# Streampunk/phaneron

Hardware: AMD Instinct MI355X
Metric: frames/sec, 4-layer 2160p50 composite pipeline (v210 unpack->CSC->combine->CSC->v210 pack) (higher is better)
Workload: dtype f32

## Files before the change

phaneron_amd/csrc/ph_kernels_lds.hip:

```cpp
#include "ph_device.h"
#include "ph_kernels.h"
#include "ph_ldslut.h"

#include <cstdlib>

#include <type_traits>

#pragma clang fp contract(off)

#ifndef PH_PROBE
#define PH_PROBE 0
#endif
#if PH_PROBE
__device__ unsigned long long g_fused_probe[2048 * 12];
extern "C" int ph_debug_fused_probe(unsigned long long *out, int n_words) {
  return (int)hipMemcpyFromSymbol(out, HIP_SYMBOL(g_fused_probe), (size_t)n_words * 8);
}
#define PH_STAMP(k)                                                                  \
  do {                                                                               \
    if (threadIdx.x == 0 && tile_begin == wg_begin) {                                \
      g_fused_probe[blockIdx.x * 12 + 2 * (k)] = __builtin_amdgcn_s_memtime();       \
      g_fused_probe[blockIdx.x * 12 + 2 * (k) + 1] = __builtin_amdgcn_s_memrealtime(); \
    }                                                                                \
  } while (0)
#else
#define PH_STAMP(k) do { } while (0)
#endif

#ifndef PH_BALANCE_WAVES
#define PH_BALANCE_WAVES 1
#endif
#if PH_BALANCE_WAVES
__device__ __forceinline__ void ph_set_wave_priority(int level) {
  switch (level) {
    case 3: __builtin_amdgcn_s_setprio(3); break;
    case 2: __builtin_amdgcn_s_setprio(2); break;
    case 1: __builtin_amdgcn_s_setprio(1); break;
    default: __builtin_amdgcn_s_setprio(0); break;
  }
}
#define PH_BALANCE(p) ph_set_wave_priority(3 - ((p) * 4) / P)
#else
#define PH_BALANCE(p) do { } while (0)
#endif

namespace ph {


__device__ __forceinline__ uint4 write_quad_lds(const float (&rgb)[18], const WriteK &wk, const LutK &lut) {
  uint32_t y[6], u[3], v[3];
#pragma unroll
  for (int j = 0; j < 6; ++j) {
    if ((j & 1) == 0) {
      const Yuv1 c = write_px_lds(rgb[3 * j], rgb[3 * j + 1], rgb[3 * j + 2], wk, lut);
      y[j] = c.y, u[j >> 1] = c.u, v[j >> 1] = c.v;
    } else {
      y[j] = write_px_luma_lds(rgb[3 * j], rgb[3 * j + 1], rgb[3 * j + 2], wk, lut);
    }
  }
  return pack_quad(y, u, v);
}

#ifndef PH_FUSED_SPLIT
#define PH_FUSED_SPLIT 0
#endif
template <int N, int P, int BS, bool PIPE = false, int MODE = 0, bool TAIL = false>
__global__ __launch_bounds__(BS) void fused_v210_combine_lds_kernel(FusedLdsArgs a, uint32_t *handoff = nullptr) {
  static_assert(!TAIL || (!PIPE && MODE == 0), "the tail instantiation exists for the shipped form only");
  const ReadK rk = load_read_k(a.f.rd_cm, a.f.rd_gm);
  const WriteK wk = load_write_k(a.f.wr_cm);
  const LutK rlut = make_lut_k(a.rd), wlut = make_lut_k(a.wr);
  const bool std_matrix = ycbcr_matrix_is_standard(rk);
  const uint32_t job = blockIdx.x / a.wg_per_job, wg_in_job = blockIdx.x - job * a.wg_per_job;
  auto layer_ptr = [&](int l) { return reinterpret_cast<const uint4 *>(job ? a.more_layers[job - 1][l] : a.f.layers[l]); };
  uint4 *const out_ptr = reinterpret_cast<uint4 *>(job ? a.more_out[job - 1] : a.f.out);
  const uint32_t per_wg = (a.f.total_quads + a.wg_per_job - 1) / a.wg_per_job;
  const uint32_t wg_begin = wg_in_job * per_wg;
  const uint32_t wg_end = wg_begin + per_wg < a.f.total_quads ? wg_begin + per_wg : a.f.total_quads;
  const uint32_t tile_quads = BS * P;
  for (uint32_t tile_begin = wg_begin; tile_begin < wg_end; tile_begin += tile_quads) {
    uint32_t st[P][9];
    auto quad_of = [&](int p) {
      const uint32_t f = tile_begin + p * BS + threadIdx.x;
      return f < wg_end ? f : wg_end - 1;
    };
    uint4 w = load_stream(layer_ptr(0) + quad_of(0));
    auto slot_kind = [&](uint32_t f) -> uint32_t {
      const uint32_t g = f - __umulhi(f, a.f.magic_qpp) * a.f.quads_per_line_pitch;
      return g < a.f.quads_per_line_used ? 0u : (g == a.f.quads_per_line_used && a.f.tail_px) ? 1u : 2u;
    };
    auto phase1_slice = [&](auto tag, uint4 w, uint32_t f, uint32_t f_next, bool more, uint32_t(&st)[9]) -> uint4 {
      const bool in_tail = TAIL && slot_kind(f) == 1u;
      const float last = TAIL ? (in_tail ? 0.0f : 1.0f) : 1.0f;
      float acc[18];
#pragma unroll
      for (int i = 0; i < 18; ++i) acc[i] = 0.0f;
#pragma unroll 1
      for (int l = 0; l < N; ++l) {
        uint4 nxt = w;
        if (l + 1 < N) nxt = load_stream(layer_ptr(l + 1) + f);
        else if (more) nxt = load_stream(layer_ptr(0) + f_next);
        const Yuv6 q = unpack_quad(w);
#pragma unroll
        for (int j = 0; j < 6; ++j) {
          const float4 t = read_px_lds<decltype(tag)::value>(q.y[j], q.cb[j >> 1], q.cr[j >> 1], rk, rlut, last);
          const float kk = 1.0f - t.w;
          asm volatile("v_fma_f32 %0, %0, %3, %4\n\tv_fma_f32 %1, %1, %3, %5\n\tv_fma_f32 %2, %2, %3, %6"
                       : "+v"(acc[3 * j]), "+v"(acc[3 * j + 1]), "+v"(acc[3 * j + 2])
                       : "v"(kk), "v"(t.x), "v"(t.y), "v"(t.z));
        }
        w = nxt;
      }
#pragma unroll
      for (int i = 0; i < 9; ++i) {
        const uint32_t lo = __float_as_uint(TAIL ? lds_lut_index_unit_tail(acc[2 * i], in_tail) : lds_lut_index_unit(acc[2 * i]));
        const uint32_t hi = __float_as_uint(TAIL ? lds_lut_index_unit_tail(acc[2 * i + 1], in_tail) : lds_lut_index_unit(acc[2 * i + 1]));
        st[i] = __builtin_amdgcn_perm(hi, lo, 0x05040100u);
        asm volatile("" : "+v"(st[i]));
      }
      return w;
    };
    PH_STAMP(0);
    if (MODE == 0 || (MODE == 1 && tile_begin == wg_begin)) {
      lds_lut_load<BS>(a.rd);
      __syncthreads();
    }
    PH_STAMP(1);
    const uint32_t tile_left = wg_end - tile_begin;
    if constexpr (PIPE) {
      auto phase1_all = [&](auto tag) {
        constexpr bool STD = decltype(tag)::value;
        auto issue_first = [&](const uint4 &word) {
          return read_px_issue<STD>((float)((word.x >> 10) & 0x3ff), (float)(word.x & 0x3ff), (float)((word.x >> 20) & 0x3ff), rk, rlut);
        };
        auto issue_px = [&](const uint4 &word, int j) {
          const uint32_t wy = j == 0 ? word.x : j < 3 ? word.y : j == 3 ? word.z : word.w;
          const uint32_t sy = (j == 0 || j == 3) ? 10u : (j == 1 || j == 4) ? 0u : 20u;
          const int pr = j >> 1;
          const uint32_t wcb = pr == 0 ? word.x : pr == 1 ? word.y : word.z, scb = 10u * pr;
          const uint32_t wcr = pr == 0 ? word.x : pr == 1 ? word.z : word.w, scr = pr == 0 ? 20u : pr == 1 ? 0u : 10u;
          return read_px_issue<STD>((float)((wy >> sy) & 0x3ff), (float)((wcb >> scb) & 0x3ff), (float)((wcr >> scr) & 0x3ff), rk, rlut);
        };
        PxPending pend = issue_first(w);
#pragma unroll
        for (int p = 0; p < P; ++p) {
          if (p * BS < tile_left) {
            PH_BALANCE(p);
            const uint32_t f = quad_of(p);
            const bool more = (p + 1 < P) && ((p + 1) * BS < tile_left);
            const uint32_t f_next = more ? quad_of(p + 1) : f;
            float acc[18];
#pragma unroll
            for (int i = 0; i < 18; ++i) acc[i] = 0.0f;
#pragma unroll 1
            for (int l = 0; l < N; ++l) {
              uint4 nxt = w;
              if (l + 1 < N) nxt = load_stream(layer_ptr(l + 1) + f);
              else if (more) nxt = load_stream(layer_ptr(0) + f_next);
#pragma unroll
              for (int j = 0; j < 6; ++j) {
                PxPending nx;
                if (j < 5) nx = issue_px(w, j + 1);
                else {
                  uint4 first = nxt;
                  asm volatile("" : "+v"(first.x));
                  nx = issue_first(first);
                }
                __builtin_amdgcn_sched_barrier(0);
                const float4 t = read_px_finish(pend, rk);
                const float kk = 1.0f - t.w;
                asm volatile("v_fma_f32 %0, %0, %3, %4\n\tv_fma_f32 %1, %1, %3, %5\n\tv_fma_f32 %2, %2, %3, %6"
                             : "+v"(acc[3 * j]), "+v"(acc[3 * j + 1]), "+v"(acc[3 * j + 2])
                             : "v"(kk), "v"(t.x), "v"(t.y), "v"(t.z));
                __builtin_amdgcn_sched_barrier(0);
                pend = nx;
              }
              w = nxt;
            }
#pragma unroll
            for (int i = 0; i < 9; ++i) {
              const uint32_t lo = __float_as_uint(lds_lut_index_unit(acc[2 * i]));
              const uint32_t hi = __float_as_uint(lds_lut_index_unit(acc[2 * i + 1]));
              st[p][i] = __builtin_amdgcn_perm(hi, lo, 0x05040100u);
              asm volatile("" : "+v"(st[p][i]));
            }
          }
        }
      };
      if (std_matrix) phase1_all(std::true_type{});
      else phase1_all(std::false_type{});
      PH_STAMP(2);
      __syncthreads();
      lds_lut_load<BS>(a.wr);
      __syncthreads();
      PH_STAMP(3);
      auto idx_at = [&](int p, int i) {
        const uint32_t v = st[p][i >> 1];
        return __uint_as_float(((i & 1) ? (v >> 16) : (v & 0xFFFFu)) | 0x4B400000u);
      };
      PxPending wp = write_px_issue(idx_at(0, 0), idx_at(0, 1), idx_at(0, 2), wlut);
#pragma unroll
      for (int p = 0; p < P; ++p) {
        if (p * BS < tile_left) {
          PH_BALANCE(p);
          const uint32_t f = tile_begin + p * BS + threadIdx.x;
          uint32_t y[6], u[3], v[3];
#pragma unroll
          for (int j = 0; j < 6; ++j) {
            PxPending nx = wp;
            if (j < 5) nx = write_px_issue(idx_at(p, 3 * j + 3), idx_at(p, 3 * j + 4), idx_at(p, 3 * j + 5), wlut);
            else if (p + 1 < P) {
              if ((p + 1) * BS < tile_left) nx = write_px_issue(idx_at(p + 1 < P ? p + 1 : p, 0), idx_at(p + 1 < P ? p + 1 : p, 1), idx_at(p + 1 < P ? p + 1 : p, 2), wlut);
            }
            __builtin_amdgcn_sched_barrier(0);
            const float gr = lds_lut_finish(wp.r), gg = lds_lut_finish(wp.g), gb = lds_lut_finish(wp.b);
            y[j] = sat_u16_rte(dot4(gr, gg, gb, 1.0f, wk.y));
            if ((j & 1) == 0) {
              u[j >> 1] = sat_u16_rte(dot4(gr, gg, gb, 1.0f, wk.u));
              v[j >> 1] = sat_u16_rte(dot4(gr, gg, gb, 1.0f, wk.v));
            }
            __builtin_amdgcn_sched_barrier(0);
            wp = nx;
          }
          if (f < wg_end) store_stream(out_ptr + f, pack_quad(y, u, v));
        }
      }
    } else {
    const uint32_t wave_first = (uint32_t)__builtin_amdgcn_readfirstlane((int)(threadIdx.x & ~63u));
    if (MODE != 2) {
#pragma unroll
    for (int p = 0; p < P; ++p) {
      const uint32_t f = quad_of(p);
      if (p * BS + wave_first < wg_end - tile_begin) {
        PH_BALANCE(p);
        const bool more = (p + 1 < P) && ((p + 1) * BS + wave_first < wg_end - tile_begin);
        const uint32_t f_next = more ? quad_of(p + 1) : f;
        if (std_matrix) w = phase1_slice(std::true_type{}, w, f, f_next, more, st[p]);
        else w = phase1_slice(std::false_type{}, w, f, f_next, more, st[p]);
      }
    }
    }
    if (MODE == 1) {
#pragma unroll
      for (int p = 0; p < P; ++p)
        if (p * BS + wave_first < wg_end - tile_begin) {
          const uint32_t f = quad_of(p);
#pragma unroll
          for (int i = 0; i < 9; ++i) handoff[(size_t)i * a.f.total_quads + f] = st[p][i];
        }
      continue;
    }
    if (MODE == 2) {
#pragma unroll
      for (int p = 0; p < P; ++p)
        if (p * BS + wave_first < wg_end - tile_begin) {
          const uint32_t f = quad_of(p);
#pragma unroll
          for (int i = 0; i < 9; ++i) st[p][i] = __builtin_nontemporal_load(handoff + (size_t)i * a.f.total_quads + f);
        }
    }
    PH_STAMP(2);
    if (MODE == 0 || tile_begin == wg_begin) {
      __syncthreads();
      lds_lut_load<BS>(a.wr);
      __syncthreads();
    }
    PH_STAMP(3);
#pragma unroll
    for (int p = 0; p < P; ++p) {
      const uint32_t f = tile_begin + p * BS + threadIdx.x;
      if (p * BS + wave_first < wg_end - tile_begin) {
        PH_BALANCE(p);
        float yi[18];
#pragma unroll
        for (int i = 0; i < 9; ++i) {
          yi[2 * i] = __uint_as_float((st[p][i] & 0xFFFFu) | 0x4B400000u);
          yi[2 * i + 1] = __uint_as_float((st[p][i] >> 16) | 0x4B400000u);
        }
        uint4 packed;
        if (TAIL) {
          const uint32_t kind = slot_kind(f < wg_end ? f : wg_end - 1);
          if (kind == 0u) packed = write_quad_idx_lds(yi, wk, wlut);
          else if (kind == 1u) packed = write_quad_idx_lds_tail(yi, wk, wlut, a.f.tail_px);
          else packed = make_uint4(0u, 0u, 0u, 0u);
        } else {
          packed = write_quad_idx_lds(yi, wk, wlut);
        }
        if (f < wg_end) store_stream(out_ptr + f, packed);
      }
    }
    }
    PH_STAMP(4);
    __syncthreads();
  }
}

__global__ __launch_bounds__(kLdsBlock) void v210_read_lds_kernel(const uint4 *__restrict__ in, float4 *__restrict__ out,
                                                                   uint32_t width, uint32_t quads_per_line_pitch,
                                                                   uint32_t total_px, const float *__restrict__ cm,
                                                                   const float *__restrict__ gm, LutView lut, uint32_t nt) {
  const ReadK k = load_read_k(cm, gm);
  const LutK lk = make_lut_k(lut);
  lds_lut_load(lut);
  __syncthreads();
  const uint32_t tail_from = width - width % 6u;
  for (uint32_t p = blockIdx.x * kLdsBlock + threadIdx.x; p < total_px; p += gridDim.x * kLdsBlock) {
    const uint32_t line = p / width, x = p - line * width;
    const uint32_t g = x / 6, j = x - 6 * g, pr = j >> 1;
    const uint4 w = in[(size_t)line * quads_per_line_pitch + g];
    const uint32_t wy = (j == 0) ? w.x : (j < 3) ? w.y : (j == 3) ? w.z : w.w;
    const uint32_t sy = (j == 0 || j == 3) ? 10u : (j == 1 || j == 4) ? 0u : 20u;
    const uint32_t wcb = pr == 0 ? w.x : pr == 1 ? w.y : w.z;
    const uint32_t wcr = pr == 0 ? w.x : pr == 1 ? w.z : w.w;
    const uint32_t scr = pr == 0 ? 20u : pr == 1 ? 0u : 10u;
    const float yf = (float)((wy >> sy) & 0x3ff);
    const float cbf = (float)((wcb >> (10u * pr)) & 0x3ff);
    const float crf = (float)((wcr >> scr) & 0x3ff);
    store_image(out + p, read_px_lds(yf, cbf, crf, k, lk, x < tail_from ? 1.0f : 0.0f), nt);
  }
}

struct ReadBatchArgs {
  const uint4 *in[kMaxLayers];
  float4 *out[kMaxLayers];
  uint32_t wg_per_frame;
};
__global__ __launch_bounds__(kLdsBlock) void v210_read_lds_batch_kernel(ReadBatchArgs a, uint32_t width, uint32_t quads_per_line_pitch,
                                                                         uint32_t total_px, const float *__restrict__ cm,
                                                                         const float *__restrict__ gm, LutView lut, uint32_t nt) {
  const ReadK k = load_read_k(cm, gm);
  const LutK lk = make_lut_k(lut);
  lds_lut_load(lut);
  __syncthreads();
  const uint32_t frame = blockIdx.x / a.wg_per_frame, wg = blockIdx.x - frame * a.wg_per_frame;
  const uint4 *__restrict__ in = a.in[frame];
  float4 *__restrict__ out = a.out[frame];
  const uint32_t tail_from = width - width % 6u;
  for (uint32_t p = wg * kLdsBlock + threadIdx.x; p < total_px; p += a.wg_per_frame * kLdsBlock) {
    const uint32_t line = p / width, x = p - line * width;
    const uint32_t g = x / 6, j = x - 6 * g, pr = j >> 1;
    const uint4 w = in[(size_t)line * quads_per_line_pitch + g];
    const uint32_t wy = (j == 0) ? w.x : (j < 3) ? w.y : (j == 3) ? w.z : w.w;
    const uint32_t sy = (j == 0 || j == 3) ? 10u : (j == 1 || j == 4) ? 0u : 20u;
    const uint32_t wcb = pr == 0 ? w.x : pr == 1 ? w.y : w.z;
    const uint32_t wcr = pr == 0 ? w.x : pr == 1 ? w.z : w.w;
    const uint32_t scr = pr == 0 ? 20u : pr == 1 ? 0u : 10u;
    const float yf = (float)((wy >> sy) & 0x3ff);
    const float cbf = (float)((wcb >> (10u * pr)) & 0x3ff);
    const float crf = (float)((wcr >> scr) & 0x3ff);
    store_image(out + p, read_px_lds(yf, cbf, crf, k, lk, x < tail_from ? 1.0f : 0.0f), nt);
  }
}

__global__ __launch_bounds__(kLdsBlock) void v210_write_lds_kernel(const float4 *__restrict__ in, uint4 *__restrict__ out,
                                                                    uint32_t width, uint32_t quads_per_line,
                                                                    uint32_t lines, uint32_t first_line,
                                                                    uint32_t line_step, const float *__restrict__ cm,
                                                                    LutView lut) {
  const WriteK k = load_write_k(cm);
  const LutK lk = make_lut_k(lut);
  lds_lut_load(lut);
  __syncthreads();
  const uint32_t total = quads_per_line * lines, full = width / 6u, remain = width - 6u * full;
  for (uint32_t f = blockIdx.x * kLdsBlock + threadIdx.x; f < total; f += gridDim.x * kLdsBlock) {
    const uint32_t li = f / quads_per_line, g = f - li * quads_per_line;
    const uint32_t line = first_line + li * line_step;
    if (g > full || (g == full && !remain)) {
      store_stream(out + (size_t)line * quads_per_line + g, make_uint4(0u, 0u, 0u, 0u));
      continue;
    }
    const float4 *row = in + (size_t)line * width;
    float rgb[18];
#pragma unroll
    for (int j = 0; j < 6; ++j) {
      const uint32_t x = 6u * g + (uint32_t)j < width ? 6u * g + (uint32_t)j : width - 1u;
      const float4 p = row[x];
// ... 360 lines not shown
  for (int l = 0; l < a.n; ++l) {
    const uint64_t bytes = (uint64_t)a.lw[l] * (uint64_t)a.lh[l] * 16u, pitch = (uint64_t)a.lw[l] * 16u;
    if (bytes + 2 * pitch > 0x80000000ull || pitch >= (1u << 23) || a.lh[l] >= (1 << 22)) return false;
    sampled = sampled || a.matrix[l] != nullptr;
  }
  for (int l = 0; l < a.n; ++l) sampled = sampled || a.wipe_with[l] != nullptr;
  return sampled;
}
static bool compose_stage_fits(const ComposeArgs &a) { return ((a.wr.bytes + 15u) & ~15u) + kComposeStageBytes <= 160u * 1024u; }
static bool compose_quad_forced() {
  static const int quad_env = [] {
    const char *e = getenv("PH_COMPOSE_QUAD");
    return e ? atoi(e) : 0;
  }();
  return quad_env != 0;
}
static bool compose_taps_enabled() {
  static const int taps_env = [] {
    const char *e = getenv("PH_COMPOSE_TAPS");
    return e ? atoi(e) : 1;
  }();
  return taps_env != 0;
}
static bool compose_uses_taps(const ComposeArgs &a) {
  return !compose_quad_forced() && compose_stage_fits(a) && compose_taps_enabled() && compose_taps_eligible(a);
}
bool compose_can_wipe(const ComposeArgs &a) { return compose_uses_taps(a); }

template <int N, bool ALL_DIRECT>
static hipError_t launch_compose_px_nd(hipStream_t s, const ComposeArgs &a, uint32_t grid, uint32_t stage_off) {
  hipError_t e = hipFuncSetAttribute(reinterpret_cast<const void *>(compose_write_v210_px_kernel<N, ALL_DIRECT>),
                                     hipFuncAttributeMaxDynamicSharedMemorySize, kMaxDynamicLds);
  if (e != hipSuccess) return e;
  compose_write_v210_px_kernel<N, ALL_DIRECT><<<grid, kLdsBlock, stage_off + kComposeStageBytes, s>>>(a, stage_off);
  return hipGetLastError();
}
template <int N>
static hipError_t launch_compose_px_n(hipStream_t s, const ComposeArgs &a, uint32_t grid, uint32_t stage_off) {
  bool all_direct = true;
  for (int l = 0; l < N; ++l) all_direct = all_direct && a.matrix[l] == nullptr;
  return all_direct ? launch_compose_px_nd<N, true>(s, a, grid, stage_off) : launch_compose_px_nd<N, false>(s, a, grid, stage_off);
}

template <typename K>
static hipError_t allow_lds(K kernel, uint32_t bytes) {
  return hipFuncSetAttribute(reinterpret_cast<const void *>(kernel), hipFuncAttributeMaxDynamicSharedMemorySize, kMaxDynamicLds);
}

#if PH_FUSED_SPLIT
template <int N, int P, int BS, int MODE>
static hipError_t launch_fused_half(hipStream_t s, FusedLdsArgs b, uint32_t lds) {
  static uint32_t *handoff = nullptr;
  static size_t handoff_quads = 0;
  if (handoff_quads < b.f.total_quads) {
    if (handoff) hipFree(handoff);
    if (hipMalloc(&handoff, (size_t)b.f.total_quads * 36) != hipSuccess) return hipErrorOutOfMemory;
    handoff_quads = b.f.total_quads;
  }
  hipError_t e = allow_lds(fused_v210_combine_lds_kernel<N, P, BS, false, MODE>, lds);
  if (e != hipSuccess) return e;
  fused_v210_combine_lds_kernel<N, P, BS, false, MODE><<<b.wg_per_job * b.jobs, BS, lds, s>>>(b, handoff);
  return hipGetLastError();
}
#endif

template <int N, int P, int BS, bool PIPE = false, bool TAIL = false>
static hipError_t launch_fused_npb(hipStream_t s, const FusedLdsArgs &a, uint32_t grid_in, uint32_t lds) {
  uint32_t grid = grid_in;
#if PH_FUSED_SPLIT
  static const int cus_env = [] {
    const char *e = getenv("PH_FUSED_CUS");
    return e ? atoi(e) : 0;
  }();
  if (cus_env > 0 && (uint32_t)cus_env < grid) grid = (uint32_t)cus_env;
#endif
  hipError_t e = allow_lds(fused_v210_combine_lds_kernel<N, P, BS, PIPE, 0, TAIL>, lds);
  if (e != hipSuccess) return e;
  const uint32_t slices = (a.f.total_quads + BS - 1) / BS;
  FusedLdsArgs b = a;
  if (b.jobs < 1) b.jobs = 1;
  b.wg_per_job = grid / b.jobs ? grid / b.jobs : 1;
  if (b.wg_per_job > slices) b.wg_per_job = slices;
#if PH_FUSED_SPLIT
  if (!PIPE && N == 4) {
    static const int mode_env = [] {
      const char *e = getenv("PH_FUSED_MODE");
      return e ? atoi(e) : 0;
    }();
    if (mode_env == 1) return launch_fused_half<N, P, BS, 1>(s, b, lds);
    if (mode_env == 2) return launch_fused_half<N, P, BS, 2>(s, b, lds);
    if (mode_env == 3) {
      hipError_t e1 = launch_fused_half<N, P, BS, 1>(s, b, lds);
      return e1 != hipSuccess ? e1 : launch_fused_half<N, P, BS, 2>(s, b, lds);
    }
  }
#endif
  fused_v210_combine_lds_kernel<N, P, BS, PIPE, 0, TAIL><<<b.wg_per_job * b.jobs, BS, lds, s>>>(b);
  return hipGetLastError();
}

template <int N>
static hipError_t launch_fused_n(hipStream_t s, const FusedLdsArgs &a, uint32_t grid, uint32_t lds) {
  static const int geom_env = [] {
    const char *e = getenv("PH_FUSED_GEOM");
    return e ? atoi(e) : 0;
  }();
  if (a.f.quads_per_line_used != a.f.quads_per_line_pitch) return launch_fused_npb<N, 6, 1024, false, true>(s, a, grid, lds);
  int geom = geom_env ? geom_env : 6;
  static const int pipe_env = [] {
    const char *e = getenv("PH_FUSED_PIPE");
    return e ? atoi(e) : 0;
  }();
#ifdef PH_FUSED_EXPERIMENT
  static const int bs_env = [] {
    const char *e = getenv("PH_FUSED_BS");
    return e ? atoi(e) : 0;
  }();
  if (N == 4 && bs_env == 768) return pipe_env ? launch_fused_npb<4, 8, 768, true>(s, a, grid, lds) : launch_fused_npb<4, 8, 768>(s, a, grid, lds);
  if (N == 4 && bs_env == 512) return pipe_env ? launch_fused_npb<4, 11, 512, true>(s, a, grid, lds) : launch_fused_npb<4, 11, 512>(s, a, grid, lds);
#endif
  if (pipe_env && geom == 6) return launch_fused_npb<N, 6, 1024, true>(s, a, grid, lds);
  if (geom == 4) return launch_fused_npb<N, 4, 1024>(s, a, grid, lds);
  if (geom == 8) return launch_fused_npb<N, 8, 1024>(s, a, grid, lds);
  return launch_fused_npb<N, 6, 1024>(s, a, grid, lds);
}

hipError_t launch_fused_v210_combine_lds(hipStream_t s, int n, const FusedLdsArgs &a, uint32_t num_cus) {
  const uint32_t lds = a.rd.bytes > a.wr.bytes ? a.rd.bytes : a.wr.bytes;
  switch (n) {
    case 1: return launch_fused_n<1>(s, a, num_cus, lds);
    case 2: return launch_fused_n<2>(s, a, num_cus, lds);
    case 3: return launch_fused_n<3>(s, a, num_cus, lds);
    case 4: return launch_fused_n<4>(s, a, num_cus, lds);
    case 5: return launch_fused_n<5>(s, a, num_cus, lds);
    case 6: return launch_fused_n<6>(s, a, num_cus, lds);
    case 7: return launch_fused_n<7>(s, a, num_cus, lds);
    case 8: return launch_fused_n<8>(s, a, num_cus, lds);
    default: return hipErrorInvalidValue;
  }
}

hipError_t launch_compose_write_v210(hipStream_t s, const ComposeArgs &a, uint32_t num_cus) {
  const uint32_t total = (a.out_w + 47u) / 48u * 8u * a.lines;
  if (!total) return hipSuccess;
  bool any_wipe = false;
  for (int l = 0; l < a.n; ++l) any_wipe = any_wipe || a.wipe_with[l] != nullptr;
  if (any_wipe && !compose_uses_taps(a)) return hipErrorInvalidValue;
  const uint32_t stage_off = (a.wr.bytes + 15u) & ~15u;
  if (!compose_quad_forced() && compose_stage_fits(a) && a.out_w % 48u == 0) {
    const uint32_t chunks = (a.out_w * a.lines + kComposeChunk - 1) / kComposeChunk;
    const uint32_t want = (chunks + kLdsBlock / 64 - 1) / (kLdsBlock / 64);
    const uint32_t grid = want < num_cus ? want : num_cus;
    if (compose_uses_taps(a)) {
      switch (a.n) {
        case 1: return launch_compose_taps_n<1>(s, a, grid, stage_off);
        case 2: return launch_compose_taps_n<2>(s, a, grid, stage_off);
        case 3: return launch_compose_taps_n<3>(s, a, grid, stage_off);
        case 4: return launch_compose_taps_n<4>(s, a, grid, stage_off);
        case 5: return launch_compose_taps_n<5>(s, a, grid, stage_off);
        case 6: return launch_compose_taps_n<6>(s, a, grid, stage_off);
        case 7: return launch_compose_taps_n<7>(s, a, grid, stage_off);
        case 8: return launch_compose_taps_n<8>(s, a, grid, stage_off);
        default: return hipErrorInvalidValue;
      }
    }
    switch (a.n) {
      case 1: return launch_compose_px_n<1>(s, a, grid, stage_off);
      case 2: return launch_compose_px_n<2>(s, a, grid, stage_off);
      case 3: return launch_compose_px_n<3>(s, a, grid, stage_off);
      case 4: return launch_compose_px_n<4>(s, a, grid, stage_off);
      case 5: return launch_compose_px_n<5>(s, a, grid, stage_off);
      case 6: return launch_compose_px_n<6>(s, a, grid, stage_off);
      case 7: return launch_compose_px_n<7>(s, a, grid, stage_off);
      case 8: return launch_compose_px_n<8>(s, a, grid, stage_off);
      default: return hipErrorInvalidValue;
    }
  }
  hipError_t e = allow_lds(compose_write_v210_kernel, a.wr.bytes);
  if (e != hipSuccess) return e;
  const uint32_t want = (total + kLdsBlock - 1) / kLdsBlock;
  compose_write_v210_kernel<<<want < num_cus ? want : num_cus, kLdsBlock, a.wr.bytes, s>>>(a);
  return hipGetLastError();
}

__global__ void lds_base_probe_kernel(uint32_t *out) {
  *out = (uint32_t)(uintptr_t)(__attribute__((address_space(3))) unsigned char *)g_lds;
}
hipError_t launch_lds_base_probe(hipStream_t s, uint32_t *out_dev) {
  lds_base_probe_kernel<<<1, 64, 16, s>>>(out_dev);
  return hipGetLastError();
}

hipError_t launch_v210_read_lds(hipStream_t s, const void *in, void *out, uint32_t width, uint32_t height,
                                const void *cm, const void *gm, const LutView &lut, uint32_t num_cus) {
  hipError_t e = allow_lds(v210_read_lds_kernel, lut.bytes);
  if (e != hipSuccess) return e;
  const uint32_t total = width * height;
  const uint32_t want = (total + kLdsBlock - 1) / kLdsBlock;
  v210_read_lds_kernel<<<want < num_cus ? want : num_cus, kLdsBlock, lut.bytes, s>>>(
      (const uint4 *)in, (float4 *)out, width, v210_pitch_bytes(width) / 16, total, (const float *)cm, (const float *)gm,
      lut, image_nt((size_t)width * height * 16));
  return hipGetLastError();
// ... 33 lines not shown
```

phaneron_amd/csrc/ph_ldslut.h:

```cpp
#pragma once
#include "ph_device.h"
#include "ph_lut.h"

#pragma clang fp contract(off)

namespace ph {

constexpr int kLdsBlock = 1024;

#ifndef PH_ABLATE
#define PH_ABLATE 0
#endif

extern __shared__ __attribute__((aligned(16))) unsigned char g_lds[];

template <int BS = kLdsBlock, bool WAIT = true>
__device__ __forceinline__ void lds_lut_load(const LutView &v) {
#if PH_ABLATE & 2
  return;
#endif
  const uint32_t n = (v.bytes - v.hole) / 16;
  unsigned char *const dst = g_lds + v.hole;
  const uint32_t wave = threadIdx.x >> 6, lane = threadIdx.x & 63;
  const uint4 *src = reinterpret_cast<const uint4 *>(v.blob);
  for (uint32_t base = wave * 64; base < n; base += BS) {
    const uint32_t i = base + lane;
    if (i < n)
      __builtin_amdgcn_global_load_lds((const __attribute__((address_space(1))) void *)(src + i),
                                       (__attribute__((address_space(3))) void *)(dst + 16 * base), 16, 0, 0);
  }
  if (WAIT) asm volatile("s_waitcnt vmcnt(0)" ::: "memory");
}

struct LutK {
  float a_scale, a_base;
  float delta_scale, delta_base;
  uint32_t a_shift;
};
typedef const __attribute__((address_space(3))) uint32_t *lds_u32_ptr;
typedef const __attribute__((address_space(3))) uint16_t *lds_u16_ptr;
__device__ __forceinline__ LutK make_lut_k(const LutView &v) {
  const uint32_t lds0 = (uint32_t)(uintptr_t)(__attribute__((address_space(3))) unsigned char *)g_lds;
  const float small = (v.delta_base + __uint_as_float(lds0)) + v.bias * v.delta_scale;
  const float b = small - kRoundMagic * v.delta_scale;
  return LutK{v.a_scale, -((kRoundMagic - v.bias) * v.a_scale), v.delta_scale, b, v.shift - 2u};
}
__device__ __forceinline__ uint32_t lds_lut_anchor_addr(const LutK &k, float y) {
  return (__float_as_uint(fma_rn(y, k.a_scale, k.a_base)) >> k.a_shift) & ~3u;
}
__device__ __forceinline__ float lds_lut_fetch(const LutK &k, float y) {
  const uint32_t a_addr = lds_lut_anchor_addr(k, y);
  const uint32_t d_addr = __float_as_uint(fma_rn(y, k.delta_scale, k.delta_base));
#if PH_ABLATE & 8
  const uint32_t a = *(lds_u32_ptr)(a_addr & 4u);
  const uint32_t d = *(lds_u16_ptr)(d_addr & 2u);
#elif PH_ABLATE & 1
  const uint32_t a = a_addr, d = d_addr;
#elif PH_ABLATE & 4
  const uint32_t a = *(lds_u32_ptr)a_addr, d = d_addr;
#else
  const uint32_t a = *(lds_u32_ptr)a_addr;
  const uint32_t d = *(lds_u16_ptr)d_addr;
#endif
#if PH_ABLATE & 16
  {
    uint32_t t;
    asm volatile("v_and_or_b32 %0, %1, %2, %3\n\tv_fma_f32 %0, %0, %0, %0\n\tv_sub_f32 %0, %0, %1\n\tv_fma_f32 %0, %0, %1, %0\n\tv_add_u32 %0, %0, %2"
                 : "=&v"(t)
                 : "v"(a), "v"(d), "v"(a_addr));
  }
#endif
  return __uint_as_float(a + d);
}
struct LutPending {
  uint32_t a, d;
};
__device__ __forceinline__ LutPending lds_lut_issue(const LutK &k, float y) {
  const uint32_t a_addr = lds_lut_anchor_addr(k, y);
  const uint32_t d_addr = __float_as_uint(fma_rn(y, k.delta_scale, k.delta_base));
#if PH_ABLATE & 8
  return LutPending{*(lds_u32_ptr)(a_addr & 4u), *(lds_u16_ptr)(d_addr & 2u)};
#elif PH_ABLATE & 1
  return LutPending{a_addr, d_addr};
#else
  return LutPending{*(lds_u32_ptr)a_addr, *(lds_u16_ptr)d_addr};
#endif
}
__device__ __forceinline__ float lds_lut_finish(const LutPending &p) {
#if PH_ABLATE & 16
  {
    uint32_t t;
    asm volatile("v_and_or_b32 %0, %1, %2, %1\n\tv_fma_f32 %0, %0, %0, %0\n\tv_sub_f32 %0, %0, %1\n\tv_fma_f32 %0, %0, %1, %0\n\tv_add_u32 %0, %0, %2"
                 : "=&v"(t)
                 : "v"(p.a), "v"(p.d));
  }
#endif
  return __uint_as_float(p.a + p.d);
}

__device__ __forceinline__ float lds_lut_index_unit(float t) {
  t = __builtin_fminf(__builtin_fmaxf(t, 0.0f), 1.0f);
  return t * 65535.0f + kRoundMagic;
}
__device__ __forceinline__ float lds_lut_index_unit_tail(float t, bool trunc) {
  t = __builtin_fminf(__builtin_fmaxf(t, 0.0f), 1.0f);
  const float x = t * 65535.0f;
  return (trunc ? __builtin_floorf(x) : x) + kRoundMagic;
}
__device__ __forceinline__ float lds_lut_at(const LutK &k, float x) {
  x = __builtin_fminf(__builtin_fmaxf(x, 0.0f), 65535.0f);
  return lds_lut_fetch(k, x + kRoundMagic);
}
__device__ __forceinline__ float lds_lut_at_unit(const LutK &k, float t) {
  return lds_lut_fetch(k, lds_lut_index_unit(t));
}

__device__ __forceinline__ uint4 write_quad_idx_lds(const float (&yi)[18], const WriteK &wk, const LutK &lut) {
  uint32_t y[6], u[3], v[3];
#pragma unroll
  for (int j = 0; j < 6; ++j) {
    const float gr = lds_lut_fetch(lut, yi[3 * j]), gg = lds_lut_fetch(lut, yi[3 * j + 1]);
    const float gb = lds_lut_fetch(lut, yi[3 * j + 2]);
    y[j] = sat_u16_rte(dot4(gr, gg, gb, 1.0f, wk.y));
    if ((j & 1) == 0) {
      u[j >> 1] = sat_u16_rte(dot4(gr, gg, gb, 1.0f, wk.u));
      v[j >> 1] = sat_u16_rte(dot4(gr, gg, gb, 1.0f, wk.v));
    }
  }
  return pack_quad(y, u, v);
}

__device__ __forceinline__ uint4 write_quad_idx_lds_tail(const float (&yi)[18], const WriteK &wk, const LutK &lut, uint32_t remain) {
  uint32_t y[4], u[2], v[2];
#pragma unroll
  for (int j = 0; j < 4; ++j) {
    const float gr = lds_lut_fetch(lut, yi[3 * j]), gg = lds_lut_fetch(lut, yi[3 * j + 1]);
    const float gb = lds_lut_fetch(lut, yi[3 * j + 2]);
    y[j] = sat_u16_trunc(__builtin_roundf(dot4(gr, gg, gb, 1.0f, wk.y)));
    if ((j & 1) == 0) {
      u[j >> 1] = sat_u16_trunc(__builtin_roundf(dot4(gr, gg, gb, 1.0f, wk.u)));
      v[j >> 1] = sat_u16_trunc(__builtin_roundf(dot4(gr, gg, gb, 1.0f, wk.v)));
    }
  }
  uint4 w = make_uint4(v[0] << 20 | y[0] << 10 | u[0], 0u, 0u, 0u);
  if (remain == 2u) {
    w.y = y[1];
  } else if (remain == 4u) {
    w.y = y[2] << 20 | u[1] << 10 | y[1];
    w.z = y[3] << 10 | v[1];
  }
  return w;
}

struct LutInLds {
  LutK k;
  __device__ __forceinline__ float at(float x) const { return lds_lut_at(k, x); }
  __device__ __forceinline__ float at_unit(float t) const { return lds_lut_at_unit(k, t); }
};
struct LutInGlobal {
  const float *__restrict__ t;
  __device__ __forceinline__ float at(float x) const { return t[sat_u16_rte(x)]; }
  __device__ __forceinline__ float at_unit(float u) const { return t[sat_u16_rte(u * 65535.0f)]; }
};

__device__ __forceinline__ bool ycbcr_matrix_is_standard(const ReadK &k) {
  return k.r.y == 0.0f && k.b.z == 0.0f && k.r.x == k.g.x && k.g.x == k.b.x;
}
template <bool STD = false>
__device__ __forceinline__ float4 read_px_lds(float y, float cb, float cr, const ReadK &k, const LutK &lut, float last = 1.0f) {
  float tr, tg, tb;
  if (STD) {
    const float ym = y * k.r.x;
    tr = fma_rn(last, k.r.w, fma_rn(cr, k.r.z, ym));
    tg = fma_rn(last, k.g.w, fma_rn(cr, k.g.z, fma_rn(cb, k.g.y, ym)));
    tb = fma_rn(last, k.b.w, fma_rn(cb, k.b.y, ym));
  } else {
    tr = dot4(y, cb, cr, last, k.r), tg = dot4(y, cb, cr, last, k.g), tb = dot4(y, cb, cr, last, k.b);
  }
  const float r = lds_lut_at_unit(lut, tr);
  const float g = lds_lut_at_unit(lut, tg);
  const float b = lds_lut_at_unit(lut, tb);
  return make_float4(dot3(r, g, b, k.gm[0], k.gm[1], k.gm[2]), dot3(r, g, b, k.gm[3], k.gm[4], k.gm[5]),
                     dot3(r, g, b, k.gm[6], k.gm[7], k.gm[8]), 1.0f);
}

struct PxPending {
  LutPending r, g, b;
};
template <bool STD>
__device__ __forceinline__ PxPending read_px_issue(float y, float cb, float cr, const ReadK &k, const LutK &lut, float last = 1.0f) {
  float tr, tg, tb;
  if (STD) {
    const float ym = y * k.r.x;
    tr = fma_rn(last, k.r.w, fma_rn(cr, k.r.z, ym));
    tg = fma_rn(last, k.g.w, fma_rn(cr, k.g.z, fma_rn(cb, k.g.y, ym)));
    tb = fma_rn(last, k.b.w, fma_rn(cb, k.b.y, ym));
  } else {
    tr = dot4(y, cb, cr, last, k.r), tg = dot4(y, cb, cr, last, k.g), tb = dot4(y, cb, cr, last, k.b);
  }
  PxPending p;
  p.r = lds_lut_issue(lut, lds_lut_index_unit(tr));
  p.g = lds_lut_issue(lut, lds_lut_index_unit(tg));
  p.b = lds_lut_issue(lut, lds_lut_index_unit(tb));
  return p;
}
__device__ __forceinline__ float4 read_px_finish(const PxPending &p, const ReadK &k) {
  const float r = lds_lut_finish(p.r), g = lds_lut_finish(p.g), b = lds_lut_finish(p.b);
  return make_float4(dot3(r, g, b, k.gm[0], k.gm[1], k.gm[2]), dot3(r, g, b, k.gm[3], k.gm[4], k.gm[5]),
                     dot3(r, g, b, k.gm[6], k.gm[7], k.gm[8]), 1.0f);
}
__device__ __forceinline__ PxPending write_px_issue(float yr, float yg, float yb, const LutK &lut) {
  PxPending p;
  p.r = lds_lut_issue(lut, yr), p.g = lds_lut_issue(lut, yg), p.b = lds_lut_issue(lut, yb);
  return p;
}

__device__ __forceinline__ Yuv1 write_px_lds(float r, float g, float b, const WriteK &k, const LutK &lut) {
  const float gr = lds_lut_at_unit(lut, r);
  const float gg = lds_lut_at_unit(lut, g);
  const float gb = lds_lut_at_unit(lut, b);
  Yuv1 o;
  o.y = sat_u16_rte(dot4(gr, gg, gb, 1.0f, k.y));
  o.u = sat_u16_rte(dot4(gr, gg, gb, 1.0f, k.u));
  o.v = sat_u16_rte(dot4(gr, gg, gb, 1.0f, k.v));
  return o;
}
__device__ __forceinline__ uint32_t write_px_luma_lds(float r, float g, float b, const WriteK &k, const LutK &lut) {
  const float gr = lds_lut_at_unit(lut, r);
  const float gg = lds_lut_at_unit(lut, g);
  const float gb = lds_lut_at_unit(lut, b);
  return sat_u16_rte(dot4(gr, gg, gb, 1.0f, k.y));
}

}
```

Before: 19670.

## Enable software-pipelined fused kernel with split LUT address/issue and wave-uniform bounds

Splits the LDS LUT lookup into an address-computation step and a load-issue step, so the next pixel's LDS reads are issued while the current pixel's finished lookups are consumed. Both phases are restructured this way, with register pinning to enforce the order, and the per-slice bounds check becomes wave-uniform. It also makes the pipelined variant the default, reuses chroma values across luma pixel pairs, and allows the split-mode path with PIPE. The costs are higher register pressure and reliance on fragile inline-asm ordering barriers.

```diff
diff --git a/phaneron_amd/csrc/ph_kernels_lds.hip b/phaneron_amd/csrc/ph_kernels_lds.hip
--- a/phaneron_amd/csrc/ph_kernels_lds.hip
+++ b/phaneron_amd/csrc/ph_kernels_lds.hip
@@ -66,7 +66,8 @@
 #endif
 template <int N, int P, int BS, bool PIPE = false, int MODE = 0, bool TAIL = false>
 __global__ __launch_bounds__(BS) void fused_v210_combine_lds_kernel(FusedLdsArgs a, uint32_t *handoff = nullptr) {
-  static_assert(!TAIL || (!PIPE && MODE == 0), "the tail instantiation exists for the shipped form only");
+  static_assert(!TAIL || (!PIPE && MODE == 0), "the tail instantiation exists for the unskewed form only");
+  static_assert(!PIPE || MODE == 0, "the skewed phases exist for the whole kernel only");
   const ReadK rk = load_read_k(a.f.rd_cm, a.f.rd_gm);
   const WriteK wk = load_write_k(a.f.wr_cm);
   const LutK rlut = make_lut_k(a.rd), wlut = make_lut_k(a.wr);
@@ -126,104 +127,119 @@
       __syncthreads();
     }
     PH_STAMP(1);
-    const uint32_t tile_left = wg_end - tile_begin;
     if constexpr (PIPE) {
-      auto phase1_all = [&](auto tag) {
-        constexpr bool STD = decltype(tag)::value;
-        auto issue_first = [&](const uint4 &word) {
-          return read_px_issue<STD>((float)((word.x >> 10) & 0x3ff), (float)(word.x & 0x3ff), (float)((word.x >> 20) & 0x3ff), rk, rlut);
-        };
-        auto issue_px = [&](const uint4 &word, int j) {
-          const uint32_t wy = j == 0 ? word.x : j < 3 ? word.y : j == 3 ? word.z : word.w;
-          const uint32_t sy = (j == 0 || j == 3) ? 10u : (j == 1 || j == 4) ? 0u : 20u;
+      const uint32_t wave_first = (uint32_t)__builtin_amdgcn_readfirstlane((int)(threadIdx.x & ~63u));
+      const uint32_t left = wg_end - tile_begin;
+      auto pin_addr = [](PxAddr &x) { asm volatile("" : "+v"(x.r.a), "+v"(x.r.d), "+v"(x.g.a), "+v"(x.g.d), "+v"(x.b.a), "+v"(x.b.d)); };
+      auto pin_pend = [](PxPending &x) { asm volatile("" : "+v"(x.r.a), "+v"(x.r.d), "+v"(x.g.a), "+v"(x.g.d), "+v"(x.b.a), "+v"(x.b.d)); };
+      float cbf = 0.0f, crf = 0.0f;
+      auto front = [&](auto tag, const uint4 &word, int j) {
+        const uint32_t wy = j == 0 ? word.x : j < 3 ? word.y : j == 3 ? word.z : word.w;
+        const uint32_t sy = (j == 0 || j == 3) ? 10u : (j == 1 || j == 4) ? 0u : 20u;
+        if ((j & 1) == 0) {
           const int pr = j >> 1;
           const uint32_t wcb = pr == 0 ? word.x : pr == 1 ? word.y : word.z, scb = 10u * pr;
           const uint32_t wcr = pr == 0 ? word.x : pr == 1 ? word.z : word.w, scr = pr == 0 ? 20u : pr == 1 ? 0u : 10u;
-          return read_px_issue<STD>((float)((wy >> sy) & 0x3ff), (float)((wcb >> scb) & 0x3ff), (float)((wcr >> scr) & 0x3ff), rk, rlut);
-        };
-        PxPending pend = issue_first(w);
-#pragma unroll
-        for (int p = 0; p < P; ++p) {
-          if (p * BS < tile_left) {
-            PH_BALANCE(p);
-            const uint32_t f = quad_of(p);
-            const bool more = (p + 1 < P) && ((p + 1) * BS < tile_left);
-            const uint32_t f_next = more ? quad_of(p + 1) : f;
-            float acc[18];
-#pragma unroll
-            for (int i = 0; i < 18; ++i) acc[i] = 0.0f;
+          cbf = (float)((wcb >> scb) & 0x3ff), crf = (float)((wcr >> scr) & 0x3ff);
+        }
+        return read_px_addr<decltype(tag)::value>((float)((wy >> sy) & 0x3ff), cbf, crf, rk, rlut);
+      };
+      PxPending pend;
+      auto phase1_skew_slice = [&](auto tag, int p) {
+        const uint32_t f = quad_of(p);
+        const bool more = (p + 1 < P) && ((p + 1) * BS + wave_first < left);
+        const uint32_t f_next = more ? quad_of(p + 1) : f;
+        float acc[18];
+#pragma unroll
+        for (int i = 0; i < 18; ++i) acc[i] = 0.0f;
 #pragma unroll 1
-            for (int l = 0; l < N; ++l) {
-              uint4 nxt = w;
-              if (l + 1 < N) nxt = load_stream(layer_ptr(l + 1) + f);
-              else if (more) nxt = load_stream(layer_ptr(0) + f_next);
-#pragma unroll
-              for (int j = 0; j < 6; ++j) {
-                PxPending nx;
-                if (j < 5) nx = issue_px(w, j + 1);
-                else {
-                  uint4 first = nxt;
-                  asm volatile("" : "+v"(first.x));
-                  nx = issue_first(first);
-                }
-                __builtin_amdgcn_sched_barrier(0);
-                const float4 t = read_px_finish(pend, rk);
-                const float kk = 1.0f - t.w;
-                asm volatile("v_fma_f32 %0, %0, %3, %4\n\tv_fma_f32 %1, %1, %3, %5\n\tv_fma_f32 %2, %2, %3, %6"
-                             : "+v"(acc[3 * j]), "+v"(acc[3 * j + 1]), "+v"(acc[3 * j + 2])
-                             : "v"(kk), "v"(t.x), "v"(t.y), "v"(t.z));
-                __builtin_amdgcn_sched_barrier(0);
-                pend = nx;
-              }
-              w = nxt;
+        for (int l = 0; l < N; ++l) {
+          uint4 nxt = w;
+          if (l + 1 < N) nxt = load_stream(layer_ptr(l + 1) + f);
+          else if (more) nxt = load_stream(layer_ptr(0) + f_next);
+#pragma unroll
+          for (int j = 0; j < 6; ++j) {
+            PxAddr at;
+            if (j < 5) at = front(tag, w, j + 1);
+            else {
+              uint4 first = nxt;
+              asm volatile("" : "+v"(first.x));
+              at = front(tag, first, 0);
             }
-#pragma unroll
-            for (int i = 0; i < 9; ++i) {
-              const uint32_t lo = __float_as_uint(lds_lut_index_unit(acc[2 * i]));
-              const uint32_t hi = __float_as_uint(lds_lut_index_unit(acc[2 * i + 1]));
-              st[p][i] = __builtin_amdgcn_perm(hi, lo, 0x05040100u);
-              asm volatile("" : "+v"(st[p][i]));
-            }
+            pin_addr(at);
+            pin_pend(pend);
+            float r = lds_lut_finish(pend.r), g = lds_lut_finish(pend.g), b = lds_lut_finish(pend.b);
+            asm volatile("" : "+v"(r), "+v"(g), "+v"(b), "+v"(at.r.a), "+v"(at.r.d), "+v"(at.g.a), "+v"(at.g.d), "+v"(at.b.a), "+v"(at.b.d), "+v"(w.x), "+v"(w.y), "+v"(w.z), "+v"(w.w));
+            pend = px_issue(at);
+            const float4 t = make_float4(dot3(r, g, b, rk.gm[0], rk.gm[1], rk.gm[2]), dot3(r, g, b, rk.gm[3], rk.gm[4], rk.gm[5]),
+                                         dot3(r, g, b, rk.gm[6], rk.gm[7], rk.gm[8]), 1.0f);
+            const float kk = 1.0f - t.w;
+            asm volatile("v_fma_f32 %0, %0, %3, %4\n\tv_fma_f32 %1, %1, %3, %5\n\tv_fma_f32 %2, %2, %3, %6"
+                         : "+v"(acc[3 * j]), "+v"(acc[3 * j + 1]), "+v"(acc[3 * j + 2])
+                         : "v"(kk), "v"(t.x), "v"(t.y), "v"(t.z));
           }
+          w = nxt;
+        }
+#pragma unroll
+        for (int i = 0; i < 9; ++i) {
+          const uint32_t lo = __float_as_uint(lds_lut_index_unit(acc[2 * i]));
+          const uint32_t hi = __float_as_uint(lds_lut_index_unit(acc[2 * i + 1]));
+          st[p][i] = __builtin_amdgcn_perm(hi, lo, 0x05040100u);
+          asm volatile("" : "+v"(st[p][i]));
         }
       };
-      if (std_matrix) phase1_all(std::true_type{});
-      else phase1_all(std::false_type{});
+      if (std_matrix) pend = px_issue(front(std::true_type{}, w, 0));
+      else pend = px_issue(front(std::false_type{}, w, 0));
+#pragma unroll
+      for (int p = 0; p < P; ++p) {
+        if (!(p * BS + wave_first < left)) break;
+        PH_BALANCE(p);
+        if (std_matrix) phase1_skew_slice(std::true_type{}, p);
+        else phase1_skew_slice(std::false_type{}, p);
+      }
       PH_STAMP(2);
       __syncthreads();
       lds_lut_load<BS>(a.wr);
       __syncthreads();
       PH_STAMP(3);
-      auto idx_at = [&](int p, int i) {
-        const uint32_t v = st[p][i >> 1];
-        return __uint_as_float(((i & 1) ? (v >> 16) : (v & 0xFFFFu)) | 0x4B400000u);
+      auto wfront = [&](uint32_t s0, uint32_t s1, int i) {
+        auto idx = [&](int k) {
+          const uint32_t v = (k >> 1) == (i >> 1) ? s0 : s1;
+          return __uint_as_float(((k & 1) ? (v >> 16) : (v & 0xFFFFu)) | 0x4B400000u);
+        };
+        return write_px_addr(idx(i), idx(i + 1), idx(i + 2), wlut);
       };
-      PxPending wp = write_px_issue(idx_at(0, 0), idx_at(0, 1), idx_at(0, 2), wlut);
+      PxAddr at = wfront(st[0][0], st[0][1], 0);
+      pend = px_issue(at);
 #pragma unroll
       for (int p = 0; p < P; ++p) {
-        if (p * BS < tile_left) {
-          PH_BALANCE(p);
-          const uint32_t f = tile_begin + p * BS + threadIdx.x;
-          uint32_t y[6], u[3], v[3];
-#pragma unroll
-          for (int j = 0; j < 6; ++j) {
-            PxPending nx = wp;
-            if (j < 5) nx = write_px_issue(idx_at(p, 3 * j + 3), idx_at(p, 3 * j + 4), idx_at(p, 3 * j + 5), wlut);
-            else if (p + 1 < P) {
-              if ((p + 1) * BS < tile_left) nx = write_px_issue(idx_at(p + 1 < P ? p + 1 : p, 0), idx_at(p + 1 < P ? p + 1 : p, 1), idx_at(p + 1 < P ? p + 1 : p, 2), wlut);
-            }
-            __builtin_amdgcn_sched_barrier(0);
-            const float gr = lds_lut_finish(wp.r), gg = lds_lut_finish(wp.g), gb = lds_lut_finish(wp.b);
-            y[j] = sat_u16_rte(dot4(gr, gg, gb, 1.0f, wk.y));
-            if ((j & 1) == 0) {
-              u[j >> 1] = sat_u16_rte(dot4(gr, gg, gb, 1.0f, wk.u));
-              v[j >> 1] = sat_u16_rte(dot4(gr, gg, gb, 1.0f, wk.v));
-            }
-            __builtin_amdgcn_sched_barrier(0);
-            wp = nx;
+        if (!(p * BS + wave_first < left)) break;
+        PH_BALANCE(p);
+        const uint32_t f = tile_begin + p * BS + threadIdx.x;
+        constexpr int kLast = P - 1;
+        const int pn = p < kLast ? p + 1 : p;
+        const bool more = (p + 1 < P) && ((p + 1) * BS + wave_first < left);
+        uint32_t y[6], u[3], v[3];
+#pragma unroll
+        for (int j = 0; j < 6; ++j) {
+          if (j < 5) at = wfront(st[p][(3 * j + 3) >> 1], st[p][(3 * j + 5) >> 1], 3 * j + 3);
+          else if (more) at = wfront(st[pn][0], st[pn][1], 0);
+          pin_addr(at);
+          pin_pend(pend);
+          float gr = lds_lut_finish(pend.r), gg = lds_lut_finish(pend.g), gb = lds_lut_finish(pend.b);
+          if (j < 4) asm volatile("" : "+v"(gr), "+v"(gg), "+v"(gb), "+v"(at.r.a), "+v"(at.r.d), "+v"(at.g.a), "+v"(at.g.d), "+v"(at.b.a), "+v"(at.b.d), "+v"(st[p][(3 * j + 6) >> 1]), "+v"(st[p][(3 * j + 8) >> 1]));
+          else asm volatile("" : "+v"(gr), "+v"(gg), "+v"(gb), "+v"(at.r.a), "+v"(at.r.d), "+v"(at.g.a), "+v"(at.g.d), "+v"(at.b.a), "+v"(at.b.d));
+          pend = px_issue(at);
+          y[j] = sat_u16_rte(dot4(gr, gg, gb, 1.0f, wk.y));
+          if ((j & 1) == 0) {
+            u[j >> 1] = sat_u16_rte(dot4(gr, gg, gb, 1.0f, wk.u));
+            v[j >> 1] = sat_u16_rte(dot4(gr, gg, gb, 1.0f, wk.v));
+            asm volatile("" : "+v"(y[j]), "+v"(u[j >> 1]), "+v"(v[j >> 1]));
+          } else {
+            asm volatile("" : "+v"(y[j]));
           }
-          if (f < wg_end) store_stream(out_ptr + f, pack_quad(y, u, v));
-        }
+        }
+        if (f < wg_end) store_stream(out_ptr + f, pack_quad(y, u, v));
       }
     } else {
     const uint32_t wave_first = (uint32_t)__builtin_amdgcn_readfirstlane((int)(threadIdx.x & ~63u));
@@ -818,7 +834,7 @@
   b.wg_per_job = grid / b.jobs ? grid / b.jobs : 1;
   if (b.wg_per_job > slices) b.wg_per_job = slices;
 #if PH_FUSED_SPLIT
-  if (!PIPE && N == 4) {
+  if (N == 4) {
     static const int mode_env = [] {
       const char *e = getenv("PH_FUSED_MODE");
       return e ? atoi(e) : 0;
@@ -845,15 +861,15 @@
   int geom = geom_env ? geom_env : 6;
   static const int pipe_env = [] {
     const char *e = getenv("PH_FUSED_PIPE");
-    return e ? atoi(e) : 0;
+    return e ? atoi(e) : 1;
   }();
 #ifdef PH_FUSED_EXPERIMENT
   static const int bs_env = [] {
     const char *e = getenv("PH_FUSED_BS");
     return e ? atoi(e) : 0;
   }();
-  if (N == 4 && bs_env == 768) return pipe_env ? launch_fused_npb<4, 8, 768, true>(s, a, grid, lds) : launch_fused_npb<4, 8, 768>(s, a, grid, lds);
-  if (N == 4 && bs_env == 512) return pipe_env ? launch_fused_npb<4, 11, 512, true>(s, a, grid, lds) : launch_fused_npb<4, 11, 512>(s, a, grid, lds);
+  if (N == 4 && bs_env == 768) return launch_fused_npb<4, 8, 768>(s, a, grid, lds);
+  if (N == 4 && bs_env == 512) return launch_fused_npb<4, 11, 512>(s, a, grid, lds);
 #endif
   if (pipe_env && geom == 6) return launch_fused_npb<N, 6, 1024, true>(s, a, grid, lds);
   if (geom == 4) return launch_fused_npb<N, 4, 1024>(s, a, grid, lds);
diff --git a/phaneron_amd/csrc/ph_ldslut.h b/phaneron_amd/csrc/ph_ldslut.h
--- a/phaneron_amd/csrc/ph_ldslut.h
+++ b/phaneron_amd/csrc/ph_ldslut.h
@@ -75,17 +75,22 @@
 struct LutPending {
   uint32_t a, d;
 };
-__device__ __forceinline__ LutPending lds_lut_issue(const LutK &k, float y) {
-  const uint32_t a_addr = lds_lut_anchor_addr(k, y);
-  const uint32_t d_addr = __float_as_uint(fma_rn(y, k.delta_scale, k.delta_base));
+struct LutAddr {
+  uint32_t a, d;
+};
+__device__ __forceinline__ LutAddr lds_lut_addr(const LutK &k, float y) {
+  return LutAddr{lds_lut_anchor_addr(k, y), __float_as_uint(fma_rn(y, k.delta_scale, k.delta_base))};
+}
+__device__ __forceinline__ LutPending lds_lut_issue(const LutAddr &at) {
 #if PH_ABLATE & 8
-  return LutPending{*(lds_u32_ptr)(a_addr & 4u), *(lds_u16_ptr)(d_addr & 2u)};
+  return LutPending{*(lds_u32_ptr)(at.a & 4u), *(lds_u16_ptr)(at.d & 2u)};
 #elif PH_ABLATE & 1
-  return LutPending{a_addr, d_addr};
+  return LutPending{at.a, at.d};
 #else
-  return LutPending{*(lds_u32_ptr)a_addr, *(lds_u16_ptr)d_addr};
-#endif
-}
+  return LutPending{*(lds_u32_ptr)at.a, *(lds_u16_ptr)at.d};
+#endif
+}
+__device__ __forceinline__ LutPending lds_lut_issue(const LutK &k, float y) { return lds_lut_issue(lds_lut_addr(k, y)); }
 __device__ __forceinline__ float lds_lut_finish(const LutPending &p) {
 #if PH_ABLATE & 16
   {
@@ -187,6 +192,36 @@
 struct PxPending {
   LutPending r, g, b;
 };
+struct PxAddr {
+  LutAddr r, g, b;
+};
+__device__ __forceinline__ PxPending px_issue(const PxAddr &at) {
+  PxPending p;
+  p.r = lds_lut_issue(at.r), p.g = lds_lut_issue(at.g), p.b = lds_lut_issue(at.b);
+  return p;
+}
+template <bool STD>
+__device__ __forceinline__ PxAddr read_px_addr(float y, float cb, float cr, const ReadK &k, const LutK &lut) {
+  float tr, tg, tb;
+  if (STD) {
+    const float ym = y * k.r.x;
+    tr = fma_rn(1.0f, k.r.w, fma_rn(cr, k.r.z, ym));
+    tg = fma_rn(1.0f, k.g.w, fma_rn(cr, k.g.z, fma_rn(cb, k.g.y, ym)));
+    tb = fma_rn(1.0f, k.b.w, fma_rn(cb, k.b.y, ym));
+  } else {
+    tr = dot4(y, cb, cr, 1.0f, k.r), tg = dot4(y, cb, cr, 1.0f, k.g), tb = dot4(y, cb, cr, 1.0f, k.b);
+  }
+  PxAddr at;
+  at.r = lds_lut_addr(lut, lds_lut_index_unit(tr));
+  at.g = lds_lut_addr(lut, lds_lut_index_unit(tg));
+  at.b = lds_lut_addr(lut, lds_lut_index_unit(tb));
+  return at;
+}
+__device__ __forceinline__ PxAddr write_px_addr(float yr, float yg, float yb, const LutK &lut) {
+  PxAddr at;
+  at.r = lds_lut_addr(lut, yr), at.g = lds_lut_addr(lut, yg), at.b = lds_lut_addr(lut, yb);
+  return at;
+}
 template <bool STD>
 __device__ __forceinline__ PxPending read_px_issue(float y, float cb, float cr, const ReadK &k, const LutK &lut, float last = 1.0f) {
   float tr, tg, tb;
```

Measured after the change: 19710, median of 5. Within noise of the previous version (+0.2%).

## Issue LDS LUT load before constant setup and load constants via scalar path

Applied to the files above, without the earlier changes.

Starts the LDS lookup-table load (without its internal wait) at kernel entry for MODE 0, then fetches the colour matrices through constant address-space pointers so they can use scalar loads. An explicit vmcnt wait is placed before the barrier, and the trailing barrier on the last tile is dropped. The aim is to overlap LUT fetch latency with setup work and trim redundant synchronisation. It relies on inline waitcnt being correct with respect to the LUT load, and on there being no LDS hazard at kernel exit.

```diff
diff --git a/phaneron_amd/csrc/ph_kernels_lds.hip b/phaneron_amd/csrc/ph_kernels_lds.hip
--- a/phaneron_amd/csrc/ph_kernels_lds.hip
+++ b/phaneron_amd/csrc/ph_kernels_lds.hip
@@ -46,6 +46,25 @@
 
 namespace ph {
 
+typedef const __attribute__((address_space(4))) float *const_f32_ptr;
+__device__ __forceinline__ ReadK load_read_k_const(const float *cm_, const float *gm_) {
+  const const_f32_ptr cm = (const_f32_ptr)cm_, gm = (const_f32_ptr)gm_;
+  ReadK k;
+  k.r = make_float4(cm[0], cm[1], cm[2], cm[3]);
+  k.g = make_float4(cm[4], cm[5], cm[6], cm[7]);
+  k.b = make_float4(cm[8], cm[9], cm[10], cm[11]);
+#pragma unroll
+  for (int i = 0; i < 9; ++i) k.gm[i] = gm[i];
+  return k;
+}
+__device__ __forceinline__ WriteK load_write_k_const(const float *cm_) {
+  const const_f32_ptr cm = (const_f32_ptr)cm_;
+  WriteK k;
+  k.y = make_float4(cm[0], cm[1], cm[2], cm[3]);
+  k.u = make_float4(cm[4], cm[5], cm[6], cm[7]);
+  k.v = make_float4(cm[8], cm[9], cm[10], cm[11]);
+  return k;
+}
 
 __device__ __forceinline__ uint4 write_quad_lds(const float (&rgb)[18], const WriteK &wk, const LutK &lut) {
   uint32_t y[6], u[3], v[3];
@@ -67,8 +86,10 @@
 template <int N, int P, int BS, bool PIPE = false, int MODE = 0, bool TAIL = false>
 __global__ __launch_bounds__(BS) void fused_v210_combine_lds_kernel(FusedLdsArgs a, uint32_t *handoff = nullptr) {
   static_assert(!TAIL || (!PIPE && MODE == 0), "the tail instantiation exists for the shipped form only");
-  const ReadK rk = load_read_k(a.f.rd_cm, a.f.rd_gm);
-  const WriteK wk = load_write_k(a.f.wr_cm);
+  constexpr bool DMA_FIRST = MODE == 0;
+  if (DMA_FIRST) lds_lut_load<BS, false>(a.rd);
+  const ReadK rk = load_read_k_const(a.f.rd_cm, a.f.rd_gm);
+  const WriteK wk = load_write_k_const(a.f.wr_cm);
   const LutK rlut = make_lut_k(a.rd), wlut = make_lut_k(a.wr);
   const bool std_matrix = ycbcr_matrix_is_standard(rk);
   const uint32_t job = blockIdx.x / a.wg_per_job, wg_in_job = blockIdx.x - job * a.wg_per_job;
@@ -78,6 +99,7 @@
   const uint32_t wg_begin = wg_in_job * per_wg;
   const uint32_t wg_end = wg_begin + per_wg < a.f.total_quads ? wg_begin + per_wg : a.f.total_quads;
   const uint32_t tile_quads = BS * P;
+  if (DMA_FIRST && wg_begin >= wg_end) asm volatile("s_waitcnt vmcnt(0)" ::: "memory");
   for (uint32_t tile_begin = wg_begin; tile_begin < wg_end; tile_begin += tile_quads) {
     uint32_t st[P][9];
     auto quad_of = [&](int p) {
@@ -122,7 +144,8 @@
     };
     PH_STAMP(0);
     if (MODE == 0 || (MODE == 1 && tile_begin == wg_begin)) {
-      lds_lut_load<BS>(a.rd);
+      if (!DMA_FIRST || tile_begin != wg_begin) lds_lut_load<BS, false>(a.rd);
+      asm volatile("s_waitcnt vmcnt(0)" ::: "memory");
       __syncthreads();
     }
     PH_STAMP(1);
@@ -291,7 +314,7 @@
     }
     }
     PH_STAMP(4);
-    __syncthreads();
+    if (tile_begin + tile_quads < wg_end) __syncthreads();
   }
 }
 
```

Result: no change. 19980 before, 20070 after (median of 6 runs) (+0.5%).
